# Danya-Is/re2-modification

Measured on AMD Instinct MI355X. Metric: input GB/s (chars matched/sec) on 10-example attack corpus, higher is better.
Workload: dtype u8

## Files before the change

### re2-modification_amd/csrc/regions.hip

```cpp
#include <hip/hip_runtime.h>
#include <hip/hip_ext.h>

#include <cstdint>
#include <cstdlib>

#include "mfa_internal.h"

namespace mfa {

static constexpr int kCleanMin = 4;
static constexpr uint32_t kMaxLen = 0x00ffffffu;

__device__ __forceinline__ uint32_t nz8(uint64_t d) {
    const uint64_t x = (((d & 0x7f7f7f7f7f7f7f7full) + 0x7f7f7f7f7f7f7f7full) | d) & 0x8080808080808080ull;
    return (uint32_t)(((x >> 7) * 0x0102040810204080ull) >> 56);
}

__device__ __forceinline__ uint64_t shr_bytes(uint64_t lo, uint64_t hi, uint32_t s) {
    return s == 0u ? lo : (s >= 8u ? hi : (lo >> (8u * s)) | (hi << (64u - 8u * s)));
}

__device__ __forceinline__ uint64_t qsad(uint32_t src_lo, uint32_t src_hi, uint32_t ref, uint64_t acc) {
    return __builtin_amdgcn_qsad_pk_u16_u8(((uint64_t)src_hi << 32) | src_lo, ref, acc);
}
__device__ __forceinline__ uint32_t pk_nz(uint32_t d) {
    uint32_t r;
    asm("v_pk_min_u16 %0, %1, %2" : "=v"(r) : "v"(d), "v"(0x00010001u));
    return r;
}

__device__ __forceinline__ constexpr uint32_t qbit(int q) {
    return q == 1 ? 1u << 16 : q == 2 ? 1u << 1 : q == 3 ? 1u << 17 : q == 4 ? 1u << 2 : q == 5 ? 1u << 18 : q == 6 ? 1u << 3 : q == 7 ? 1u << 19 : 1u << 4;
}
static constexpr uint32_t kAllDirty = 0x000f001eu;

__device__ __forceinline__ uint32_t block_mask(uint32_t w0, uint32_t w1, uint32_t w2, uint32_t w3, uint32_t w4, uint32_t w5) {
    uint64_t a = 0, b = 0;
    a = qsad(w0, w1, w0, a); a = qsad(w1, w2, w1, a); a = qsad(w2, w3, w2, a); a = qsad(w3, w4, w3, a);
    b = qsad(w1, w2, w0, b); b = qsad(w2, w3, w1, b); b = qsad(w3, w4, w2, b); b = qsad(w4, w5, w3, b);
    const uint32_t d8 = (w0 ^ w2) | (w1 ^ w3) | (w2 ^ w4) | (w3 ^ w5);
    const uint32_t z0 = pk_nz((uint32_t)a), z1 = pk_nz((uint32_t)(a >> 32)), z2 = pk_nz((uint32_t)b), z3 = pk_nz((uint32_t)(b >> 32));
    const uint32_t z8 = d8 < 1u ? d8 : 1u;
    return ((z0 | (z1 << 1)) | ((z2 << 2) | (z3 << 3)) | (z8 << 4)) & kAllDirty;
}

struct RegionState {
    int32_t  last_dirty[9];
    uint32_t ncand;
    uint32_t shortest;
    uint32_t cq;
    int32_t  cx, cy;
};

__device__ __forceinline__ uint32_t wave_min_u32(uint32_t v) {
#define MFA_DPP_MIN(ctrl, rows) { const uint32_t t = (uint32_t)__builtin_amdgcn_update_dpp((int)v, (int)v, ctrl, rows, 0xf, false); v = t < v ? t : v; }
    MFA_DPP_MIN(0x111, 0xf)
    MFA_DPP_MIN(0x112, 0xf)
    MFA_DPP_MIN(0x114, 0xf)
    MFA_DPP_MIN(0x118, 0xf)
    MFA_DPP_MIN(0x142, 0xa)
    MFA_DPP_MIN(0x143, 0xc)
#undef MFA_DPP_MIN
    return (uint32_t)__builtin_amdgcn_readlane((int)v, 63);
}
static constexpr uint32_t kEarly = 3;
__device__ __forceinline__ uint32_t shortest_candidate(const RegionState& st, uint32_t lane) {
    return wave_min_u32(lane < kEarly ? 0xffffffc0u | lane : ((uint32_t)(st.cy - st.cx) << 6) | lane);
}

template <int Q>
__device__ __forceinline__ void emit(RegionState& st, uint32_t lane, int32_t x, int32_t y) {
    if (st.ncand < 64u) {
        if (lane == st.ncand) { st.cq = Q; st.cx = x; st.cy = y; }
        st.ncand++;
        st.shortest = ~0u;
        return;
    }
    if (st.shortest == ~0u) st.shortest = shortest_candidate(st, lane);
    if ((uint32_t)(y - x) <= (st.shortest >> 6)) return;
    if (lane == (st.shortest & 63u)) { st.cq = Q; st.cx = x; st.cy = y; }
    st.shortest = ~0u;
}

template <int Q>
__device__ __forceinline__ bool book(RegionState& st, uint32_t lane, unsigned long long dirty, int32_t base) {
    int32_t& last = st.last_dirty[Q];
    if (dirty == ~0ull && last == base - 1) { last = base + 63; return false; }
    if (dirty == 0ull) return false;
    bool emitted = false;
    const int32_t first = (int32_t)__builtin_ctzll(dirty), top = 63 - (int32_t)__builtin_clzll(dirty);
    if (base + first - last - 1 >= kCleanMin) { emit<Q>(st, lane, last, base + first); emitted = true; }
    unsigned long long z = ~dirty;
    unsigned long long zz = z;
#pragma unroll
    for (int k = 1; k < kCleanMin; k++) zz &= z >> k;
    const unsigned long long inside = first < top ? ((~0ull >> (63 - top)) & (~0ull << first)) : 0ull;
    for (unsigned long long w = zz & inside; w;) {
        const int32_t s = (int32_t)__builtin_ctzll(w);
        const int32_t e = s + (int32_t)__builtin_ctzll(dirty >> s);
        emit<Q>(st, lane, base + s - 1, base + e);
        emitted = true;
        w &= ~0ull << e;
    }
    last = base + top;
    return emitted;
}

struct RowBook { unsigned long long dirty[9]; int32_t before[9]; };

template <int Q, int D>
__device__ __forceinline__ bool row_same_as(RegionState& st, RowBook& rb) {
    if constexpr (D >= Q || Q % D != 0) return false;
    else {
        if (rb.dirty[Q] != rb.dirty[D] || rb.before[Q] != rb.before[D]) return false;
        st.last_dirty[Q] = st.last_dirty[D];
        return true;
    }
}

template <int Q, int D>
__device__ __forceinline__ bool row_inside(RegionState& st, RowBook& rb, int32_t base) {
    if constexpr (D >= Q || Q % D != 0) return false;
    else {
        if ((rb.dirty[D] & ~rb.dirty[Q]) != 0ull || rb.before[Q] < rb.before[D] || rb.dirty[Q] == 0ull) return false;
        st.last_dirty[Q] = base + 63 - (int32_t)__builtin_clzll(rb.dirty[Q]);
        return true;
    }
}

template <int Q>
__device__ __forceinline__ void row_prep(RegionState& st, uint32_t mask, uint32_t settled, int32_t base, RowBook& rb) {
    if (settled & qbit(Q)) st.last_dirty[Q] = base - 1;
    rb.dirty[Q] = __ballot((mask & qbit(Q)) != 0u);
    rb.before[Q] = st.last_dirty[Q];
}
template <int Q>
__device__ __forceinline__ void row_period(RegionState& st, uint32_t lane, int32_t base, RowBook& rb) {
    if (row_inside<Q, 1>(st, rb, base)) return;
    if (row_same_as<Q, 4>(st, rb) || row_same_as<Q, 3>(st, rb) || row_same_as<Q, 2>(st, rb) || row_same_as<Q, 1>(st, rb)) return;
    if (row_inside<Q, 2>(st, rb, base) || row_inside<Q, 3>(st, rb, base) || row_inside<Q, 4>(st, rb, base)) return;
    (void)book<Q>(st, lane, rb.dirty[Q], base);
}
struct Geo {
    uint64_t a0;
    uint32_t off0, len;
    int32_t nblk, endblk, nrows;
    uint32_t lastoff, ylim;
};

__device__ __forceinline__ Geo make_geo(uint64_t b, uint64_t e, uint64_t ymax) {
    Geo g;
    g.len = (uint32_t)(e - b);
    g.a0 = b & ~(uint64_t)15;
    g.off0 = (uint32_t)(b - g.a0);
    g.nblk = (int32_t)((g.off0 + g.len + 15u) >> 4);
    g.endblk = g.len >= 8u ? (int32_t)((g.off0 + g.len - 8u) >> 4) : 0;
    g.nrows = (g.nblk + 63) >> 6;
    g.lastoff = g.nblk > 0 ? 16u * (uint32_t)(g.nblk - 1) : 0u;
    {
        const uint64_t d = ymax - g.a0;
        uint64_t top;
        asm("s_lshr_b64 %0, %1, 32" : "=s"(top) : "s"(d) : "scc");
        const uint32_t dl = (uint32_t)d;
        g.ylim = top != 0ull ? 0xfffffff0u : (dl < 0xfffffff0u ? dl : 0xfffffff0u);
    }
    return g;
}

struct Scan {
    RegionState st;
    uint32_t settled, vp;
};

__device__ __forceinline__ void scan_reset(Scan& sc) {
#pragma unroll
    for (int q = 0; q < 9; q++) sc.st.last_dirty[q] = -1;
    sc.st.ncand = 0; sc.st.shortest = ~0u; sc.st.cq = 0; sc.st.cx = 0; sc.st.cy = 0;
    sc.settled = ~0u; sc.vp = 0u;
}

typedef uint32_t u32x4 __attribute__((ext_vector_type(4)));
typedef uint32_t u32x2 __attribute__((ext_vector_type(2)));
struct Row { u32x4 x; u32x2 y; };

__device__ __forceinline__ void row_request(const uint8_t* sbase, const Geo& g, int32_t row, uint32_t lane, Row& r) {
    row = row < g.nrows ? row : g.nrows - 1;
    uint32_t off = (uint32_t)row * 1024u + 16u * lane;
    off = off < g.lastoff ? off : g.lastoff;
    uint32_t yo = off + 16u;
    yo = yo < g.ylim ? yo : g.ylim;
    asm volatile("global_load_dwordx4 %0, %1, %2" : "=&v"(r.x) : "v"(off), "s"(sbase) : "memory");
    if (lane == 63u) asm volatile("global_load_dwordx2 %0, %1, %2" : "+v"(r.y) : "v"(yo), "s"(sbase) : "memory");
}
__device__ __forceinline__ uint2 row_tail(const Row& r) {
    return make_uint2((uint32_t)__builtin_amdgcn_update_dpp((int)r.y[0], (int)r.x[0], 0x130, 0xf, 0xf, false),
                      (uint32_t)__builtin_amdgcn_update_dpp((int)r.y[1], (int)r.x[1], 0x130, 0xf, 0xf, false));
}
template <int YOUNGER, bool SAFE>
__device__ __forceinline__ void row_wait_older(Row& r) {
    if (SAFE) asm volatile("s_waitcnt vmcnt(0)" : "+v"(r.x), "+v"(r.y) :: "memory");
    else asm volatile("s_waitcnt vmcnt(%2)" : "+v"(r.x), "+v"(r.y) : "n"(2 * YOUNGER) : "memory");
}
__device__ __forceinline__ void row_wait_all(Row& r) { asm volatile("s_waitcnt vmcnt(0)" : "+v"(r.x), "+v"(r.y) :: "memory"); }

__device__ __forceinline__ void scan_row(Scan& sc, uint32_t lane, const Geo& g, const int32_t row, const uint4 x, const uint2 y) {
    RegionState& st = sc.st;
    const int32_t base = row * 64, blk = base + (int32_t)lane;
    const bool forced = blk == 0 || blk >= g.endblk;
    const uint32_t vp = sc.vp;
    if (vp != 0u) {
        uint32_t s0, s1, s2, s3;
        if (vp < 4u) {
            s0 = __builtin_amdgcn_alignbyte(x.y, x.x, vp); s1 = __builtin_amdgcn_alignbyte(x.z, x.y, vp);
            s2 = __builtin_amdgcn_alignbyte(x.w, x.z, vp); s3 = __builtin_amdgcn_alignbyte(y.x, x.w, vp);
        } else if (vp < 8u) {
            s0 = __builtin_amdgcn_alignbyte(x.z, x.y, vp - 4u); s1 = __builtin_amdgcn_alignbyte(x.w, x.z, vp - 4u);
            s2 = __builtin_amdgcn_alignbyte(y.x, x.w, vp - 4u); s3 = __builtin_amdgcn_alignbyte(y.y, y.x, vp - 4u);
        } else { s0 = x.z; s1 = x.w; s2 = y.x; s3 = y.y; }
        uint32_t diff = (x.x ^ s0) | (x.y ^ s1) | (x.z ^ s2) | (x.w ^ s3);
        if (vp < 8u) {
            const uint64_t yy = ((uint64_t)y.y << 32) | y.x;
            const uint64_t dd = (yy ^ (yy >> (8u * vp))) << (8u * vp);
            diff |= (uint32_t)dd | (uint32_t)(dd >> 32);
        }
        if (!__any(forced || diff != 0u)) return;
    }
    const uint32_t mask = forced ? kAllDirty : block_mask(x.x, x.y, x.z, x.w, y.x, y.y);
    if (__all(mask == sc.settled)) return;
    const uint32_t was = sc.settled != ~0u ? sc.settled : 0u;
    RowBook rb;
    row_prep<1>(st, mask, was, base, rb);
    (void)book<1>(st, lane, rb.dirty[1], base);
    bool inside = rb.dirty[1] != 0ull && !__any((mask & qbit(1)) != 0u && mask != kAllDirty);
    if (inside) {
        int32_t least = 0x7fffffff;
#pragma unroll
        for (int q = 2; q <= 8; q++) { const int32_t bq = (was & qbit(q)) ? base - 1 : st.last_dirty[q]; least = bq < least ? bq : least; }
        inside = least >= rb.before[1];
    }
    if (inside) {
#pragma unroll
        for (int q = 2; q <= 8; q++) st.last_dirty[q] = base + 63;
    } else {
        row_prep<2>(st, mask, was, base, rb); row_period<2>(st, lane, base, rb);
        row_prep<3>(st, mask, was, base, rb); row_period<3>(st, lane, base, rb);
        row_prep<4>(st, mask, was, base, rb); row_period<4>(st, lane, base, rb);
        row_prep<5>(st, mask, was, base, rb); row_period<5>(st, lane, base, rb);
        row_prep<6>(st, mask, was, base, rb); row_period<6>(st, lane, base, rb);
        row_prep<7>(st, mask, was, base, rb); row_period<7>(st, lane, base, rb);
        row_prep<8>(st, mask, was, base, rb); row_period<8>(st, lane, base, rb);
    }
    const int32_t b63 = base + 63;
    sc.settled = (b63 < g.endblk) ? (uint32_t)__builtin_amdgcn_readlane((int)mask, 63) : ~0u;
    const uint32_t clean = ~sc.settled;
    const uint32_t vo = 2u * (uint32_t)__builtin_ctz(((clean >> 16) & 0xfu) | 0x10u) + 1u, ve = 2u * (uint32_t)__builtin_ctz(((clean >> 1) & 0xfu) | 0x10u) + 2u;
    const uint32_t v = vo < ve ? vo : ve;
    sc.vp = v <= 8u ? v : 0u;
}

struct RowOut { bool entry; uint32_t rank; uint64_t word, header; };
__device__ __forceinline__ RowOut finish_string(Scan& sc, uint32_t lane, const Geo& g, const uint8_t* bytes, uint64_t total16) {
    RegionState& st = sc.st;
    const uint32_t ncand = st.ncand < 64u ? st.ncand : 64u;
    bool keep = false;
    uint32_t lo = 0, hi = 0;
    const uint32_t q = st.cq;
    if (lane < ncand) {
        const int32_t vlo = (int32_t)g.off0, vhi = (int32_t)g.off0 + (int32_t)g.len - (int32_t)q;
        const uint8_t* const sbase = bytes + g.a0;
        auto ld8 = [&](uint32_t off) -> uint64_t {
            uint64_t v = 0;
            if (off <= g.ylim) v = *reinterpret_cast<const uint64_t*>(sbase + off);
            return v;
        };
        {
            const int32_t w0 = 16 * st.cx;
            const uint64_t p0 = ld8((uint32_t)w0), p1 = ld8((uint32_t)w0 + 8u), p2 = ld8((uint32_t)w0 + 16u);
            uint32_t m = nz8(p0 ^ shr_bytes(p0, p1, q)) | (nz8(p1 ^ shr_bytes(p1, p2, q)) << 8);
            uint32_t valid = 0xffffu;
            if (vlo > w0) valid &= vlo - w0 >= 16 ? 0u : (0xffffu << (uint32_t)(vlo - w0));
            if (vhi < w0 + 16) valid &= vhi <= w0 ? 0u : (0xffffu >> (uint32_t)(w0 + 16 - vhi));
            m &= valid;
            const int32_t lo_abs = m ? w0 + (31 - __builtin_clz(m)) + 1 : (w0 > vlo ? w0 : vlo);
            lo = (uint32_t)(lo_abs - vlo);
        }
        {
            const int32_t w0 = 16 * st.cy;
            const uint64_t p0 = ld8((uint32_t)w0), p1 = ld8((uint32_t)w0 + 8u), p2 = ld8((uint32_t)w0 + 16u), p3 = ld8((uint32_t)w0 + 24u),
                           p4 = ld8((uint32_t)w0 + 32u);
            uint32_t m = nz8(p0 ^ shr_bytes(p0, p1, q)) | (nz8(p1 ^ shr_bytes(p1, p2, q)) << 8) | (nz8(p2 ^ shr_bytes(p2, p3, q)) << 16) |
                         (nz8(p3 ^ shr_bytes(p3, p4, q)) << 24);
            uint32_t valid = 0xffffffffu;
            if (vhi < w0 + 32) valid = vhi <= w0 ? 0u : (0xffffffffu >> (uint32_t)(w0 + 32 - vhi));
            m &= valid;
            int32_t hi_abs;
            if (m) hi_abs = w0 + __builtin_ctz(m) + (int32_t)q;
            else if (vhi < w0 + 32) hi_abs = vlo + (int32_t)g.len;
            else hi_abs = w0 + 32 + (int32_t)q;
            hi = (uint32_t)(hi_abs - vlo);
        }
        keep = hi > lo && hi - lo >= MFA_REGION_MIN_LEN && hi <= g.len;
    }
    for (uint32_t f = 0; f < ncand; f++) {
        const uint32_t qf = (uint32_t)__builtin_amdgcn_readlane((int)q, (int)f), lof = (uint32_t)__builtin_amdgcn_readlane((int)lo, (int)f),
                       hif = (uint32_t)__builtin_amdgcn_readlane((int)hi, (int)f);
        const bool kf = __builtin_amdgcn_readlane((int)keep, (int)f) != 0;
        if (!kf) continue;
        const bool divides = ((0x804020108824aaffull >> (((qf - 1u) * 8u + (q - 1u)) & 63u)) & 1ull) != 0ull;
        if (lane < ncand && lane != f && qf < q && divides && lof <= lo + 16u && hif + 16u >= hi) keep = false;
    }
    unsigned long long kb = __ballot(keep);
    const uint32_t total = (uint32_t)__builtin_popcountll(kb);
    if (total > MFA_REGION_MAX) {
        const uint32_t pkey = (lo << 4) | q;
        uint32_t before = 0;
        for (unsigned long long m = kb; m; m &= m - 1ull) {
            const int f = __builtin_ctzll(m);
            const uint32_t kf = (uint32_t)__builtin_amdgcn_readlane((int)pkey, f);
            if (kf < pkey || (kf == pkey && (uint32_t)f < lane)) before++;
        }
        const bool early = keep && before < kEarly;
        const unsigned long long eb = __ballot(early);
        const uint32_t mine = hi - lo;
        uint32_t longer = 0;
        for (unsigned long long m = kb & ~eb; m; m &= m - 1ull) {
            const int f = __builtin_ctzll(m);
            const uint32_t lf = (uint32_t)__builtin_amdgcn_readlane((int)mine, f);
            if (lf > mine || (lf == mine && (uint32_t)f < lane)) longer++;
        }
        keep = keep && (early || longer < MFA_REGION_MAX - (uint32_t)__builtin_popcountll(eb));
        kb = __ballot(keep);
    }
    uint32_t rank = 0;
    {
        const uint32_t key = (lo << 4) | q;
        for (unsigned long long m = kb; m; m &= m - 1ull) {
            const int f = __builtin_ctzll(m);
            const uint32_t kf = (uint32_t)__builtin_amdgcn_readlane((int)key, f);
            if (kf < key || (kf == key && (uint32_t)f < lane)) rank++;
        }
    }
    RowOut out;
    out.header = (uint64_t)(total < MFA_REGION_MAX ? total : MFA_REGION_MAX) | ((total > MFA_REGION_MAX || st.ncand >= 64u) ? MFA_REGION_OVERFLOW : 0ull);
    out.entry = keep && rank < MFA_REGION_MAX;
    out.rank = rank;
    out.word = (uint64_t)lo | ((uint64_t)hi << 24) | ((uint64_t)q << 48);
    return out;
}

__device__ __forceinline__ void row_out(uint64_t* tab, uint32_t lane, const RowOut& r) {
    if (r.entry) tab[1 + r.rank] = r.word;
    if (lane == 0) tab[0] = r.header;
}

constexpr int kRegionDepth = 2;
template <int MODE, int DEPTH, bool SAFE>
__global__ void __launch_bounds__(256, 8) region_scan_kernel(const uint8_t* __restrict__ bytes, const uint64_t* __restrict__ offsets, uint64_t n,
                                                             uint64_t* __restrict__ table, uint32_t rotate) {
    const uint32_t lane = threadIdx.x & 63u;
    const uint32_t wpb = blockDim.x >> 6;
    const uint64_t wave = (uint64_t)blockIdx.x * wpb + (uint32_t)__builtin_amdgcn_readfirstlane((int)(threadIdx.x >> 6)), n_waves = (uint64_t)gridDim.x * wpb;
    const uint64_t total16 = (offsets[n] + 15u) & ~(uint64_t)15;
    const uint64_t ymax = total16 - 8u;
    uint64_t first = wave;
    if (rotate && (wave | 63ull) < n) first = (wave & ~63ull) | ((wave + 17ull * (wave >> 6)) & 63ull);
    for (uint64_t sid = first; sid < n; sid += n_waves) {
        const uint64_t b = offsets[sid], e = offsets[sid + 1];
        uint64_t* const tab = table + sid * MFA_REGION_WORDS;
        static_assert(kMaxLen == 0x00ffffffu, "the test below is a shift");
        uint64_t over;
        asm("s_lshr_b64 %0, %1, 24" : "=s"(over) : "s"(e - b) : "scc");
        if (over != 0ull) { if (lane == 0) tab[0] = MFA_REGION_OVERFLOW; continue; }
        const Geo g = make_geo(b, e, ymax);
        const uint8_t* const sbase = bytes + g.a0;
        Scan sc;
        scan_reset(sc);
        Row r[DEPTH];
#pragma unroll
        for (int k = 0; k < DEPTH; k++) { r[k].x = u32x4{0, 0, 0, 0}; r[k].y = u32x2{0, 0}; }
        bool more = g.nrows > 0;
        if (more) {
#pragma unroll
            for (int k = 0; k < DEPTH - 1; k++) row_request(sbase, g, k, lane, r[k]);
        }
        for (int32_t row = 0; more; row += DEPTH) {
            bool go = true;
#pragma unroll
            for (int k = 0; k < DEPTH; k++) {
                if (go) {
                    row_request(sbase, g, row + k + DEPTH - 1, lane, r[(k + DEPTH - 1) % DEPTH]);
                    row_wait_older<DEPTH - 1, SAFE>(r[k]);
                    scan_row(sc, lane, g, row + k, make_uint4(r[k].x[0], r[k].x[1], r[k].x[2], r[k].x[3]), row_tail(r[k]));
                    go = row + k + 1 < g.nrows;
                }
            }
            more = go;
        }
#pragma unroll
        for (int k = 0; k < DEPTH; k++) row_wait_all(r[k]);
        if (MODE == 1) { if (lane == 0) tab[0] = sc.st.ncand; continue; }
        row_out(tab, lane, finish_string(sc, lane, g, bytes, total16));
    }
}

int launch_region_scan(int n_cus, const uint8_t* d_bytes, const uint64_t* d_offsets, uint64_t n, uint64_t* d_table, void* stream, unsigned threads, void* done_event) {
    if (n == 0) { if (done_event) HIP_TRY(hipEventRecord((hipEvent_t)done_event, (hipStream_t)stream)); return MFA_OK; }
    hipStream_t s = (hipStream_t)stream;
    const char* em = getenv("MFA_REGION_MODE");
    const int mode = em ? atoi(em) : 0;
    const uint64_t cus = (uint64_t)(n_cus > 0 ? n_cus : 256);
    const char* eb = getenv("MFA_REGION_BLOCK");
    const unsigned block = eb && (atoi(eb) == 64 || atoi(eb) == 128 || atoi(eb) == 256) ? (unsigned)atoi(eb) : (threads == 128u ? 128u : 256u);
    const uint64_t wpb = block / 64u;
    uint64_t blocks = (n + wpb - 1) / wpb;
    const uint64_t cap = cus * 8u * 64u * (4u / wpb);
    if (blocks > cap) blocks = cap;
    const char* el = getenv("MFA_REGION_LDS");
    const unsigned lds = el ? (unsigned)atoi(el) : 0u;
    const char* ed = getenv("MFA_REGION_DEPTH");
    const int depth = ed ? atoi(ed) : kRegionDepth;
    const char* er = getenv("MFA_REGION_ROTATE");
    const uint32_t rotate = er && er[0] == '0' ? 0u : 1u;
    const char* es = getenv("MFA_REGION_SAFE_WAITS");
    const bool safe = es && es[0] == '1';
    if (mode == 1) hipLaunchKernelGGL((region_scan_kernel<1, kRegionDepth, false>), dim3((unsigned)blocks), dim3(block), lds, s, d_bytes, d_offsets, n, d_table, rotate);
    else if (safe) hipLaunchKernelGGL((region_scan_kernel<0, 2, true>), dim3((unsigned)blocks), dim3(block), lds, s, d_bytes, d_offsets, n, d_table, rotate);
    else if (depth == 2 && done_event) hipExtLaunchKernelGGL((region_scan_kernel<0, 2, false>), dim3((unsigned)blocks), dim3(block), lds, s, nullptr, (hipEvent_t)done_event, 0u, d_bytes, d_offsets, n, d_table, rotate);
    else if (depth == 2) hipLaunchKernelGGL((region_scan_kernel<0, 2, false>), dim3((unsigned)blocks), dim3(block), lds, s, d_bytes, d_offsets, n, d_table, rotate);
    else if (depth == 4) hipLaunchKernelGGL((region_scan_kernel<0, 4, false>), dim3((unsigned)blocks), dim3(block), lds, s, d_bytes, d_offsets, n, d_table, rotate);
    else if (depth == 3) hipLaunchKernelGGL((region_scan_kernel<0, 3, false>), dim3((unsigned)blocks), dim3(block), lds, s, d_bytes, d_offsets, n, d_table, rotate);
    else return MFA_ERR_UNSUPPORTED;
    HIP_TRY(hipGetLastError());
    if (done_event && !(depth == 2 && mode != 1 && !safe)) HIP_TRY(hipEventRecord((hipEvent_t)done_event, s));
    return MFA_OK;
}

}
```

Baseline: 4932.

## Distribute per-period region bookkeeping across wave lanes instead of serial unrolled loop

The eight per-period dirty-run bookkeeping passes, each once an inlined template executed uniformly by the whole wave, are now handled by lanes 1-8. Each of those lanes holds its period's dirty ballot, written in with v_writelane, and its last_dirty value. Each lane runs the redundancy checks (same-as or inside a divisor period) and the run extraction in parallel, and emitted candidates are drained one at a time through a ballot loop. This is meant to cut the large serial, scalar-heavy code path and its register pressure from nine last_dirty slots, at the cost of divergent per-lane loops, readlane traffic and hand-written writelane asm with s_nop hazards.

After: 4962, median of 6. No clear change (+0.6%).

```diff
diff --git a/re2-modification_amd/csrc/region_book.h b/re2-modification_amd/csrc/region_book.h
--- /dev/null
+++ b/re2-modification_amd/csrc/region_book.h
@@ -0,0 +1,81 @@
+#ifndef MFA_REGION_BOOK_H
+#define MFA_REGION_BOOK_H
+
+#include <cstdint>
+
+#if defined(__HIPCC__)
+#define MFA_RB_FN __host__ __device__ inline __attribute__((always_inline))
+#else
+#define MFA_RB_FN inline
+#endif
+
+namespace mfa {
+
+constexpr int kCleanMin = 4;
+
+constexpr uint32_t rb_qbit(uint32_t q) { return 1u << ((q >> 1) + ((q & 1u) << 4)); }
+
+MFA_RB_FN int32_t rb_lowest(uint64_t v) { return (int32_t)__builtin_ctzll(v | (1ull << 63)); }
+MFA_RB_FN int32_t rb_highest(uint64_t v) { return 63 - (int32_t)__builtin_clzll(v | 1ull); }
+
+struct RbDiv {
+    uint64_t dirty[5];
+    int32_t before[5];
+};
+
+MFA_RB_FN bool rb_covers(uint64_t dirty_d, uint64_t dirty_q) { return (dirty_d & ~dirty_q) == 0ull; }
+MFA_RB_FN bool rb_reaches(int32_t before_q, int32_t before_d) { return before_q >= before_d; }
+
+MFA_RB_FN bool rb_same_as(uint64_t dirty_q, int32_t before_q, uint64_t dirty_d, int32_t before_d) {
+    return ((int)(dirty_q == dirty_d) & (int)(before_q == before_d)) != 0;
+}
+MFA_RB_FN bool rb_inside(uint64_t dirty_q, int32_t before_q, uint64_t dirty_d, int32_t before_d) {
+    return ((int)rb_covers(dirty_d, dirty_q) & (int)rb_reaches(before_q, before_d) & (int)(dirty_q != 0ull)) != 0;
+}
+MFA_RB_FN bool rb_inside_one(uint64_t dirty_q, int32_t before_q, uint64_t dirty_1, int32_t before_1) {
+    return ((int)rb_covers(dirty_1, dirty_q) & (int)rb_reaches(before_q, before_1)) != 0;
+}
+
+MFA_RB_FN bool rb_quiet(uint32_t q, uint64_t dirty, int32_t before, const RbDiv& d) {
+    const uint32_t divs = (uint32_t)(0xB17131100ull >> (4u * (q & 15u))) & 15u;
+    uint32_t quiet = 0u;
+    for (uint32_t D = 1; D <= 4; D++)
+        quiet |= (divs >> (D - 1u)) & ((uint32_t)rb_same_as(dirty, before, d.dirty[D], d.before[D]) | (uint32_t)rb_inside(dirty, before, d.dirty[D], d.before[D]));
+    return (quiet & 1u) != 0u;
+}
+
+struct RbRow {
+    uint64_t dirty;
+    uint64_t w;
+    int32_t base, before;
+    bool back;
+};
+
+MFA_RB_FN int32_t rb_begin(RbRow& r, uint64_t dirty, int32_t base, int32_t last, bool quiet) {
+    static_assert(kCleanMin == 4, "zz below is written for four blocks");
+    const bool some = dirty != 0ull;
+    const int32_t first = rb_lowest(dirty), top = rb_highest(dirty);
+    const uint64_t z = ~dirty;
+    uint64_t zz = z & (z >> 1);
+    zz &= zz >> 2;
+    const uint64_t inside = (~0ull >> (63 - top)) & ~(dirty ^ (dirty - 1ull));
+    r.dirty = dirty; r.base = base; r.before = last;
+    r.w = quiet ? 0ull : zz & inside;
+    r.back = ((int)some & (int)!quiet & (int)(base + first - last - 1 >= kCleanMin)) != 0;
+    return some ? base + top : last;
+}
+
+MFA_RB_FN bool rb_next(RbRow& r, int32_t& x, int32_t& y) {
+    const bool back = r.back, has = ((int)back | (int)(r.w != 0ull)) != 0;
+    const int32_t s = rb_lowest(r.w);
+    const int32_t e = (s + rb_lowest(r.dirty >> s)) & 63;
+    x = back ? r.before : r.base + s - 1;
+    y = r.base + (back ? rb_lowest(r.dirty) : e);
+    r.w = back ? r.w : r.w & (~0ull << e);
+    r.back = false;
+    return has;
+}
+
+}
+
+#endif
diff --git a/re2-modification_amd/csrc/regions.hip b/re2-modification_amd/csrc/regions.hip
--- a/re2-modification_amd/csrc/regions.hip
+++ b/re2-modification_amd/csrc/regions.hip
@@ -5,10 +5,10 @@
 #include <cstdlib>
 
 #include "mfa_internal.h"
+#include "region_book.h"
 
 namespace mfa {
 
-static constexpr int kCleanMin = 4;
 static constexpr uint32_t kMaxLen = 0x00ffffffu;
 
 __device__ __forceinline__ uint32_t nz8(uint64_t d) {
@@ -33,6 +33,8 @@
     return q == 1 ? 1u << 16 : q == 2 ? 1u << 1 : q == 3 ? 1u << 17 : q == 4 ? 1u << 2 : q == 5 ? 1u << 18 : q == 6 ? 1u << 3 : q == 7 ? 1u << 19 : 1u << 4;
 }
 static constexpr uint32_t kAllDirty = 0x000f001eu;
+static_assert(qbit(1) == rb_qbit(1) && qbit(2) == rb_qbit(2) && qbit(3) == rb_qbit(3) && qbit(4) == rb_qbit(4) && qbit(5) == rb_qbit(5) &&
+              qbit(6) == rb_qbit(6) && qbit(7) == rb_qbit(7) && qbit(8) == rb_qbit(8), "region_book.h computes a lane's bit from its number");
 
 __device__ __forceinline__ uint32_t block_mask(uint32_t w0, uint32_t w1, uint32_t w2, uint32_t w3, uint32_t w4, uint32_t w5) {
     uint64_t a = 0, b = 0;
@@ -45,7 +47,7 @@
 }
 
 struct RegionState {
-    int32_t  last_dirty[9];
+    int32_t  last_dirty;
     uint32_t ncand;
     uint32_t shortest;
     uint32_t cq;
@@ -68,79 +70,18 @@
     return wave_min_u32(lane < kEarly ? 0xffffffc0u | lane : ((uint32_t)(st.cy - st.cx) << 6) | lane);
 }
 
-template <int Q>
-__device__ __forceinline__ void emit(RegionState& st, uint32_t lane, int32_t x, int32_t y) {
+__device__ __forceinline__ void emit(RegionState& st, uint32_t lane, uint32_t q, int32_t x, int32_t y) {
+    uint32_t to = 64u;
     if (st.ncand < 64u) {
-        if (lane == st.ncand) { st.cq = Q; st.cx = x; st.cy = y; }
-        st.ncand++;
+        to = st.ncand++;
         st.shortest = ~0u;
-        return;
-    }
-    if (st.shortest == ~0u) st.shortest = shortest_candidate(st, lane);
-    if ((uint32_t)(y - x) <= (st.shortest >> 6)) return;
-    if (lane == (st.shortest & 63u)) { st.cq = Q; st.cx = x; st.cy = y; }
-    st.shortest = ~0u;
-}
-
-template <int Q>
-__device__ __forceinline__ bool book(RegionState& st, uint32_t lane, unsigned long long dirty, int32_t base) {
-    int32_t& last = st.last_dirty[Q];
-    if (dirty == ~0ull && last == base - 1) { last = base + 63; return false; }
-    if (dirty == 0ull) return false;
-    bool emitted = false;
-    const int32_t first = (int32_t)__builtin_ctzll(dirty), top = 63 - (int32_t)__builtin_clzll(dirty);
-    if (base + first - last - 1 >= kCleanMin) { emit<Q>(st, lane, last, base + first); emitted = true; }
-    unsigned long long z = ~dirty;
-    unsigned long long zz = z;
-#pragma unroll
-    for (int k = 1; k < kCleanMin; k++) zz &= z >> k;
-    const unsigned long long inside = first < top ? ((~0ull >> (63 - top)) & (~0ull << first)) : 0ull;
-    for (unsigned long long w = zz & inside; w;) {
-        const int32_t s = (int32_t)__builtin_ctzll(w);
-        const int32_t e = s + (int32_t)__builtin_ctzll(dirty >> s);
-        emit<Q>(st, lane, base + s - 1, base + e);
-        emitted = true;
-        w &= ~0ull << e;
-    }
-    last = base + top;
-    return emitted;
-}
-
-struct RowBook { unsigned long long dirty[9]; int32_t before[9]; };
-
-template <int Q, int D>
-__device__ __forceinline__ bool row_same_as(RegionState& st, RowBook& rb) {
-    if constexpr (D >= Q || Q % D != 0) return false;
-    else {
-        if (rb.dirty[Q] != rb.dirty[D] || rb.before[Q] != rb.before[D]) return false;
-        st.last_dirty[Q] = st.last_dirty[D];
-        return true;
-    }
-}
-
-template <int Q, int D>
-__device__ __forceinline__ bool row_inside(RegionState& st, RowBook& rb, int32_t base) {
-    if constexpr (D >= Q || Q % D != 0) return false;
-    else {
-        if ((rb.dirty[D] & ~rb.dirty[Q]) != 0ull || rb.before[Q] < rb.before[D] || rb.dirty[Q] == 0ull) return false;
-        st.last_dirty[Q] = base + 63 - (int32_t)__builtin_clzll(rb.dirty[Q]);
-        return true;
-    }
-}
-
-template <int Q>
-__device__ __forceinline__ void row_prep(RegionState& st, uint32_t mask, uint32_t settled, int32_t base, RowBook& rb) {
-    if (settled & qbit(Q)) st.last_dirty[Q] = base - 1;
-    rb.dirty[Q] = __ballot((mask & qbit(Q)) != 0u);
-    rb.before[Q] = st.last_dirty[Q];
-}
-template <int Q>
-__device__ __forceinline__ void row_period(RegionState& st, uint32_t lane, int32_t base, RowBook& rb) {
-    if (row_inside<Q, 1>(st, rb, base)) return;
-    if (row_same_as<Q, 4>(st, rb) || row_same_as<Q, 3>(st, rb) || row_same_as<Q, 2>(st, rb) || row_same_as<Q, 1>(st, rb)) return;
-    if (row_inside<Q, 2>(st, rb, base) || row_inside<Q, 3>(st, rb, base) || row_inside<Q, 4>(st, rb, base)) return;
-    (void)book<Q>(st, lane, rb.dirty[Q], base);
-}
+    } else {
+        if (st.shortest == ~0u) st.shortest = shortest_candidate(st, lane);
+        if ((uint32_t)(y - x) > (st.shortest >> 6)) { to = st.shortest & 63u; st.shortest = ~0u; }
+    }
+    if (lane == to) { st.cq = q; st.cx = x; st.cy = y; }
+}
+
 struct Geo {
     uint64_t a0;
     uint32_t off0, len;
@@ -173,8 +114,7 @@
 };
 
 __device__ __forceinline__ void scan_reset(Scan& sc) {
-#pragma unroll
-    for (int q = 0; q < 9; q++) sc.st.last_dirty[q] = -1;
+    sc.st.last_dirty = -1;
     sc.st.ncand = 0; sc.st.shortest = ~0u; sc.st.cq = 0; sc.st.cx = 0; sc.st.cy = 0;
     sc.settled = ~0u; sc.vp = 0u;
 }
@@ -228,30 +168,52 @@
     const uint32_t mask = forced ? kAllDirty : block_mask(x.x, x.y, x.z, x.w, y.x, y.y);
     if (__all(mask == sc.settled)) return;
     const uint32_t was = sc.settled != ~0u ? sc.settled : 0u;
-    RowBook rb;
-    row_prep<1>(st, mask, was, base, rb);
-    (void)book<1>(st, lane, rb.dirty[1], base);
-    bool inside = rb.dirty[1] != 0ull && !__any((mask & qbit(1)) != 0u && mask != kAllDirty);
-    if (inside) {
-        int32_t least = 0x7fffffff;
-#pragma unroll
-        for (int q = 2; q <= 8; q++) { const int32_t bq = (was & qbit(q)) ? base - 1 : st.last_dirty[q]; least = bq < least ? bq : least; }
-        inside = least >= rb.before[1];
-    }
-    if (inside) {
-#pragma unroll
-        for (int q = 2; q <= 8; q++) st.last_dirty[q] = base + 63;
-    } else {
-        row_prep<2>(st, mask, was, base, rb); row_period<2>(st, lane, base, rb);
-        row_prep<3>(st, mask, was, base, rb); row_period<3>(st, lane, base, rb);
-        row_prep<4>(st, mask, was, base, rb); row_period<4>(st, lane, base, rb);
-        row_prep<5>(st, mask, was, base, rb); row_period<5>(st, lane, base, rb);
-        row_prep<6>(st, mask, was, base, rb); row_period<6>(st, lane, base, rb);
-        row_prep<7>(st, mask, was, base, rb); row_period<7>(st, lane, base, rb);
-        row_prep<8>(st, mask, was, base, rb); row_period<8>(st, lane, base, rb);
-    }
-    const int32_t b63 = base + 63;
-    sc.settled = (b63 < g.endblk) ? (uint32_t)__builtin_amdgcn_readlane((int)mask, 63) : ~0u;
+    const uint32_t next_settled = (base + 63 < g.endblk) ? (uint32_t)__builtin_amdgcn_readlane((int)mask, 63) : ~0u;
+    int32_t last = st.last_dirty;
+    if (lane - 1u < 8u && (was & rb_qbit(lane & 15u)) != 0u) last = base - 1;
+    const unsigned long long d1 = __ballot((mask & qbit(1)) != 0u);
+    const int32_t before1 = __builtin_amdgcn_readlane(last, 1);
+    const bool others = lane - 2u < 7u;
+    bool inside = d1 != 0ull && !__any((mask & qbit(1)) != 0u && mask != kAllDirty);
+    if (inside) inside = !__any(others && !rb_reaches(last, before1));
+    uint32_t dlo = 0u, dhi = 0u;
+#define MFA_LO(D) "s"((uint32_t)(D))
+#define MFA_HI(D) "s"((uint32_t)((D) >> 32))
+    asm("s_nop 3\n\tv_writelane_b32 %0, %2, 1\n\tv_writelane_b32 %1, %3, 1" : "+v"(dlo), "+v"(dhi) : MFA_LO(d1), MFA_HI(d1));
+    bool quiet = false;
+    if (!inside) {
+        RbDiv dv;
+        dv.dirty[0] = 0ull; dv.before[0] = 0;
+        dv.dirty[1] = d1; dv.before[1] = before1;
+        const unsigned long long d2 = __ballot((mask & qbit(2)) != 0u), d3 = __ballot((mask & qbit(3)) != 0u), d4 = __ballot((mask & qbit(4)) != 0u),
+                                 d5 = __ballot((mask & qbit(5)) != 0u), d6 = __ballot((mask & qbit(6)) != 0u), d7 = __ballot((mask & qbit(7)) != 0u),
+                                 d8 = __ballot((mask & qbit(8)) != 0u);
+        asm("s_nop 3\n\t"
+            "v_writelane_b32 %0, %2, 2\n\tv_writelane_b32 %1, %3, 2\n\tv_writelane_b32 %0, %4, 3\n\tv_writelane_b32 %1, %5, 3\n\t"
+            "v_writelane_b32 %0, %6, 4\n\tv_writelane_b32 %1, %7, 4\n\tv_writelane_b32 %0, %8, 5\n\tv_writelane_b32 %1, %9, 5\n\t"
+            "v_writelane_b32 %0, %10, 6\n\tv_writelane_b32 %1, %11, 6\n\tv_writelane_b32 %0, %12, 7\n\tv_writelane_b32 %1, %13, 7\n\t"
+            "v_writelane_b32 %0, %14, 8\n\tv_writelane_b32 %1, %15, 8"
+            : "+v"(dlo), "+v"(dhi)
+            : MFA_LO(d2), MFA_HI(d2), MFA_LO(d3), MFA_HI(d3), MFA_LO(d4), MFA_HI(d4), MFA_LO(d5), MFA_HI(d5), MFA_LO(d6), MFA_HI(d6), MFA_LO(d7), MFA_HI(d7),
+              MFA_LO(d8), MFA_HI(d8));
+        dv.dirty[2] = d2; dv.before[2] = __builtin_amdgcn_readlane(last, 2);
+        dv.dirty[3] = d3; dv.before[3] = __builtin_amdgcn_readlane(last, 3);
+        dv.dirty[4] = d4; dv.before[4] = __builtin_amdgcn_readlane(last, 4);
+        quiet = rb_quiet(lane, ((uint64_t)dhi << 32) | dlo, last, dv);
+    }
+#undef MFA_LO
+#undef MFA_HI
+    RbRow rr;
+    last = rb_begin(rr, ((uint64_t)dhi << 32) | dlo, base, last, quiet);
+    st.last_dirty = inside && others ? base + 63 : last;
+    int32_t cx = 0, cy = 0;
+    bool has = rb_next(rr, cx, cy);
+    for (unsigned long long hb = __ballot(has); hb != 0ull; hb = __ballot(has)) {
+        const uint32_t q = (uint32_t)__builtin_ctzll(hb);
+        emit(st, lane, q, __builtin_amdgcn_readlane(cx, (int)q), __builtin_amdgcn_readlane(cy, (int)q));
+        if (lane == q) has = rb_next(rr, cx, cy);
+    }
+    sc.settled = next_settled;
     const uint32_t clean = ~sc.settled;
     const uint32_t vo = 2u * (uint32_t)__builtin_ctz(((clean >> 16) & 0xfu) | 0x10u) + 1u, ve = 2u * (uint32_t)__builtin_ctz(((clean >> 1) & 0xfu) | 0x10u) + 2u;
     const uint32_t v = vo < ve ? vo : ve;
```
